# youmi-zym/GO-SLAM

Hardware: AMD Instinct MI355X
Metric: BA keyframes/s (6 x FactorGraph.update: reproject + corr lookup + GRU + 2 GN BA iters) on synthetic 640x480 RGB-D (higher is better)
Workload: dtype f32 (BA/geometry; fp64 solve), f16 (corr volume, GRU convs); 1 GPU; configs[1]-shaped frontend window: 60x80 maps (480x640 RGB-D), P=25 keyframes, E=75 edges, 6 updates/keyframe, iters=2, RGB-D depth prior, upsample on; parallelism=replicas x1 (tracking does not shard)

## Files before the change

go_slam_amd/_lib.py:

```python
import ctypes
import os
import subprocess

_HERE = os.path.dirname(os.path.abspath(__file__))
CSRC = os.path.join(_HERE, "csrc")
LIB_PATH = os.environ.get("GOSLAM_HIP_LIB") or os.path.join(CSRC, "libgoslam_hip.so")

_lib = None

c_int, c_float, c_void_p, c_size_t = ctypes.c_int, ctypes.c_float, ctypes.c_void_p, ctypes.c_size_t

_P = c_void_p
SIGNATURES = {
    "gs_version": (ctypes.c_char_p, []),
    "gs_last_error": (ctypes.c_char_p, []),
    "gs_enc_conv_wpack_elems": (c_size_t, [c_int, c_int, c_int]),
    "gs_enc_conv_stat_chunks": (c_int, [c_int, c_int, c_int]),
    "gs_enc_conv": (c_int, [_P, c_int, c_int, _P, _P, _P, c_int, c_int, c_int, c_int, c_int, c_int, c_int, _P, _P, _P]),
    "gs_norm_act_workspace_bytes_chunks": (c_size_t, [c_int, c_int, c_int]),
    "gs_timing_begin": (c_int, [_P]),
    "gs_timing_end": (c_int, []),
    "gs_timing_read": (c_int, [ctypes.c_char_p, ctypes.POINTER(ctypes.c_double), ctypes.POINTER(c_int)]),
    "gs_timing_names": (c_int, [ctypes.c_char_p, c_int]),
    "gs_corr_index_forward": (c_int, [_P, _P, _P] + [c_int] * 7 + [_P]),
# ... 28 lines not shown
    "gs_upmask_upsample": (c_int, [_P, c_int, _P, _P, _P, _P, _P, c_int, c_int, c_int, _P]),
    "gs_bias_act": (c_int, [_P, _P, _P, c_int, c_int, c_int, c_int, c_int, _P]),
    "gs_motion_features": (c_int, [_P, _P, _P, c_int, c_int, c_int, _P]),
    "gs_ba_inputs": (c_int, [_P] * 6 + [c_int, c_int, c_int, _P]),
    "gs_lowmem_gather": (c_int, [_P] * 7 + [c_int, c_int, c_int, _P]),
    "gs_lowmem_scatter": (c_int, [_P] * 8 + [c_int, c_int, c_int, _P]),
    "gs_damping_rows": (c_int, [_P] * 5 + [c_int, c_int, c_float, c_float, _P]),
    "gs_conv1x1": (c_int, [_P, c_int, c_int, _P, _P, c_int, _P, c_int, c_int, ctypes.c_longlong, _P]),
    "gs_conv7x7_c4": (c_int, [_P, _P, _P, _P, c_int, c_int, c_int, c_int, c_int, c_int, _P]),
    "gs_conv3x3_wpack_elems": (c_size_t, [c_int, c_int]),
    "gs_conv3x3_pp": (c_int, [_P, c_int, c_int, _P, c_int, _P, c_int, c_int, c_int, c_int, c_int, c_int, _P]),
    "gs_conv3x3_bias_relu": (c_int, [_P, c_int, c_int, _P, _P, _P, c_int, c_int, c_int, c_int, c_int, _P]),
    "gs_conv3x3_gru_zr": (c_int, [_P, c_int, c_int, _P, _P, _P, _P, _P, _P, c_int, c_int, c_int, _P]),
    "gs_conv3x3_gru_zr2": (c_int, [_P, _P, c_int, c_int, _P, _P, _P, _P, _P, _P, c_int, c_int, c_int, _P]),
    "gs_conv3x3_gru_q": (c_int, [_P, _P, c_int, c_int, _P, _P, _P, _P, _P, _P, _P, c_int, c_int, c_int, _P]),
    "gs_conv3x3_head": (c_int, [_P, c_int, _P, c_int, _P, _P, c_int, c_int, c_float, _P, c_int, c_int, c_int, _P]),
    "gs_conv3x3_heads": (c_int, [_P, c_int, c_int, _P, c_int, _P, _P, c_int, _P, _P, c_int, c_int, c_int, c_int, c_int, _P]),
    "gs_conv3x3_heads_finish": (c_int, [_P, _P, _P, c_int, c_int, c_float, c_float, _P, _P, c_int, c_int, c_int, _P]),
    "gs_segment_mean": (c_int, [_P, c_int, _P, c_int, _P, _P, _P, c_int, c_int, c_int, _P]),
    "gs_norm_act_workspace_bytes": (c_size_t, [c_int, c_int, c_int]),
    "gs_norm_act": (c_int, [_P, _P, _P, _P] + [c_int] * 6 + [c_float, _P, c_size_t, c_int, _P]),
    "gs_gru_glo_workspace_bytes": (c_size_t, [c_int]),
    "gs_gru_glo": (c_int, [_P] * 11 + [c_int, c_int, _P, c_size_t, _P]),
    "gs_gru_glo_fused_workspace_bytes": (c_size_t, [c_int, c_int]),
    "gs_gru_glo_fused": (c_int, [_P, c_int] + [_P] * 10 + [c_int, c_int, _P, c_size_t, _P]),
    "gs_gru_gate_zr": (c_int, [_P] * 6 + [c_int] * 3 + [_P]),
    "gs_gru_gate_q": (c_int, [_P] * 7 + [c_int] * 2 + [_P]),
    "gs_edge_prep": (c_int, [_P] * 4 + [c_int, _P, _P] + [c_int] * 6 + [c_float, c_int, c_int, _P]),
    "gs_edge_greedy": (c_int, [_P] * 5 + [c_int] * 5 + [c_float, c_int, c_int, _P]),
    "gs_ba_workspace_bytes": (c_size_t, [c_int] * 5),
# ... 179 lines not shown
```

go_slam_amd/csrc/conv3x3_pp.hip:

```cpp
#include "common.h"
#include "conv3x3_common.h"

namespace {

constexpr int PP_KG = 4;
constexpr int PP_PSTR = 5;
constexpr int pp_zpad(int tw) { return (((2 * (tw + 2) + 2) * PP_PSTR + 3 + 15) / 16) * 16; }
constexpr int pp_patch_slots(int tw) {
  return (((512 / tw + 2) * (tw + 2) * PP_PSTR + 511) / 512) * 512 + pp_zpad(tw);
}

__device__ __attribute__((aligned(16))) const uint32_t pp_zero_page[4] = {0u, 0u, 0u, 0u};

__device__ __forceinline__ void pp_glds16(const void* src, void* lds_wave_base) {
  __builtin_amdgcn_global_load_lds((const __attribute__((address_space(1))) void*)src,
                                   (__attribute__((address_space(3))) void*)lds_wave_base, 16, 0, 0);
}

#define PP_BAR()                              \
  do {                                        \
    asm volatile("" ::: "memory");            \
    __builtin_amdgcn_s_barrier();             \
    asm volatile("" ::: "memory");            \
    __builtin_amdgcn_sched_barrier(0);        \
  } while (0)

#define PP_LGKM0()                                        \
  do {                                                    \
    asm volatile("s_waitcnt lgkmcnt(0)" ::: "memory");    \
    __builtin_amdgcn_sched_barrier(0);                    \
  } while (0)

struct PpEpi {
  const float* bias;
  const float* glo;
  const _Float16* inp_pre;
  const _Float16* aux0;
  const _Float16* aux1;
  _Float16* out0;
  _Float16* out1;
  const _Float16* xb;
  int xsb, split;
  const half8* tapw;
  float* tap_out;
  int n_tap;
  long long* dbg;
  int variant;
};

template <bool PROBE>
__device__ __forceinline__ void pp_stamp(long long* dbg, int slot) {
// ... 279 lines not shown
          }
        }
        __builtin_amdgcn_fence(__ATOMIC_RELEASE, "wavefront");
        __builtin_amdgcn_wave_barrier();
      }
      return;
    }
  }
  constexpr int PIECES = NJ * 4;
  constexpr int PXIT = 64 / PIECES;
  constexpr int NIT = 32 / PXIT;
#pragma unroll
  for (int i = 0; i < 4; ++i) {
    size_t pix4[NIT];
    bool ok4[NIT];
    half8 pi4[NIT], u4[NIT], v4[NIT];
    const int piece = lane & (PIECES - 1);
    const int c8 = wn * (PP_BN / 2) + piece * 8;
#pragma unroll
    for (int it = 0; it < NIT; ++it) {
      const int pxr = it * PXIT + lane / PIECES;
      int ty, tx;
      tile_pixel<TW, true>(wm, i, pxr, ty, tx);
      const int gv = g0 + ty, gx = tx0 + tx;
      ok4[it] = gv < rows && gx < W;
      pix4[it] = (size_t)gv * W + gx;
      if constexpr (EPI == 1 || EPI == 2) {
        const half8 z8 = {0, 0, 0, 0, 0, 0, 0, 0};
        pi4[it] = z8; u4[it] = z8; v4[it] = z8;
        if (ok4[it]) {
          if constexpr (EPI == 1) {
            if (ep.inp_pre) pi4[it] = *reinterpret_cast<const half8*>(ep.inp_pre + pix4[it] * 384 + nb * 128 + c8);
            if (nb == 1) u4[it] = *reinterpret_cast<const half8*>(x + pix4[it] * xs + c8);
          } else {
            if (ep.inp_pre) pi4[it] = *reinterpret_cast<const half8*>(ep.inp_pre + pix4[it] * 384 + 256 + c8);
            u4[it] = *reinterpret_cast<const half8*>(ep.aux0 + pix4[it] * 128 + c8);
            v4[it] = *reinterpret_cast<const half8*>(ep.aux1 + pix4[it] * 128 + c8);
          }
        }
      }
    }
#pragma unroll
    for (int j = 0; j < NJ; ++j)
#pragma unroll
      for (int g = 0; g < 4; ++g) {
        half4 o;
#pragma unroll
        for (int e = 0; e < 4; ++e) o[e] = (_Float16)acc[j][i][4 * g + e];
        *reinterpret_cast<half4*>(tile + r * PP_TS + j * 32 + 8 * g + 4 * kgl) = o;
      }
// ... 3 lines not shown
#pragma unroll
    for (int it = 0; it < NIT; ++it) {
      const int pxr = it * PXIT + lane / PIECES;
      if (ok4[it]) {
        const half8 v = *reinterpret_cast<const half8*>(tile + pxr * PP_TS + piece * 8);
        const size_t pix = pix4[it];
        if constexpr (EPI == 0 || EPI == 4) {
          *reinterpret_cast<half8*>(yb + pix * ys + piece * 8) = v;
        } else if constexpr (EPI == 3) {
          const float* bb = ep.bias + nb * PP_BN + c8;
          half8 o;
#pragma unroll
          for (int k = 0; k < 8; ++k) o[k] = (_Float16)fmaxf((float)v[k] + bb[k], 0.0f);
          *reinterpret_cast<half8*>(yb + pix * ys + piece * 8) = o;
        } else if constexpr (EPI == 1) {
          const int img = (int)(pix / ((size_t)H * W));
          const half8 pi = pi4[it];
          const float* bb = ep.bias + nb * 128 + c8;
          const float* gg = ep.glo + (size_t)img * 256 + nb * 128 + c8;
          half8 o;
          if (nb == 0) {
#pragma unroll
            for (int k = 0; k < 8; ++k) o[k] = (_Float16)pp_sigm((float)v[k] + (float)pi[k] + bb[k] + gg[k]);
            *reinterpret_cast<half8*>(ep.out0 + pix * 128 + c8) = o;
          } else {
            const half8 net = u4[it];
#pragma unroll
            for (int k = 0; k < 8; ++k)
              o[k] = (_Float16)(pp_sigm((float)v[k] + (float)pi[k] + bb[k] + gg[k]) * (float)net[k]);
            *reinterpret_cast<half8*>(ep.out1 + pix * 128 + c8) = o;
          }
        } else {
          const int img = (int)(pix / ((size_t)H * W));
          const half8 pi = pi4[it], zz = u4[it], nn = v4[it];
          const float* bb = ep.bias + c8;
          const float* gg = ep.glo + (size_t)img * 128 + c8;
          half8 o;
#pragma unroll
          for (int k = 0; k < 8; ++k) {
            const float a_ = (float)v[k] + (float)pi[k] + bb[k] + gg[k];
            const float q = gs_tanh(a_);
            const float zf = (float)zz[k];
            o[k] = (_Float16)((1.0f - zf) * (float)nn[k] + zf * q);
          }
          *reinterpret_cast<half8*>(ep.out0 + pix * 128 + c8) = o;
        }
      }
    }
// ... 62 lines not shown
  GS_REQUIRE(hx_stride >= c_in && hx_stride % 8 == 0, "conv3x3_gru_zr: bad hx_stride");
  GS_REQUIRE(n >= 0 && h > 0 && w > 0, "conv3x3_gru_zr: bad shape");
  if (n == 0) return GS_OK;
  PpEpi ep = PpEpi();
  ep.bias = bias_zr;
  ep.glo = glo_zr;
  ep.inp_pre = (const _Float16*)inp_pre;
  ep.out0 = (_Float16*)z_out;
  ep.out1 = (_Float16*)rnet_out;
  ep.xb = (const _Float16*)hx;
  ep.xsb = hx_stride;
  ep.split = 1 << 30;
  return dispatch_pp<1>(hx, hx_stride, c_in, wpack, pp_tile_width(w), nullptr, 0, 256, n, h, w, 1, (hipStream_t)stream, ep);
}

extern "C" int gs_conv3x3_gru_zr2(const void* net, const void* x_rest, int x_rest_stride, int c_rest, const void* wpack,
                                  const float* bias_zr, const float* glo_zr, const void* inp_pre, void* z_out,
                                  void* rnet_out, int n, int h, int w, gs_stream_t stream) {
  GS_REQUIRE(net && x_rest && wpack && bias_zr && glo_zr && z_out && rnet_out, "conv3x3_gru_zr2: null pointer");
  GS_REQUIRE(c_rest > 0 && c_rest % 32 == 0, "conv3x3_gru_zr2: c_rest must be a multiple of 32");
  GS_REQUIRE(x_rest_stride >= c_rest && x_rest_stride % 8 == 0, "conv3x3_gru_zr2: bad x_rest_stride");
  GS_REQUIRE(n >= 0 && h > 0 && w > 0, "conv3x3_gru_zr2: bad shape");
  if (n == 0) return GS_OK;
  PpEpi ep = PpEpi();
  ep.bias = bias_zr;
  ep.glo = glo_zr;
  ep.inp_pre = (const _Float16*)inp_pre;
  ep.out0 = (_Float16*)z_out;
  ep.out1 = (_Float16*)rnet_out;
  ep.xb = (const _Float16*)x_rest;
  ep.xsb = x_rest_stride;
  ep.split = 128;
  return dispatch_pp<1>(net, 128, 128 + c_rest, wpack, pp_tile_width(w), nullptr, 0, 256, n, h, w, 1,
                        (hipStream_t)stream, ep);
}

extern "C" int gs_conv3x3_gru_q(const void* rnet, const void* x_rest, int x_rest_stride, int c_rest, const void* wpack,
                                const float* bias_q, const float* glo_q, const void* inp_pre, const void* z,
                                const void* net, void* net_out, int n, int h, int w, gs_stream_t stream) {
  GS_REQUIRE(rnet && x_rest && wpack && bias_q && glo_q && z && net && net_out, "conv3x3_gru_q: null pointer");
  GS_REQUIRE(c_rest > 0 && c_rest % 32 == 0, "conv3x3_gru_q: c_rest must be a multiple of 32");
  GS_REQUIRE(x_rest_stride >= c_rest && x_rest_stride % 8 == 0, "conv3x3_gru_q: bad x_rest_stride");
  GS_REQUIRE(n >= 0 && h > 0 && w > 0, "conv3x3_gru_q: bad shape");
  if (n == 0) return GS_OK;
  PpEpi ep = PpEpi();
  ep.bias = bias_q;
  ep.glo = glo_q;
  ep.inp_pre = (const _Float16*)inp_pre;
  ep.aux0 = (const _Float16*)z;
  ep.aux1 = (const _Float16*)net;
  ep.out0 = (_Float16*)net_out;
  ep.xb = (const _Float16*)x_rest;
  ep.xsb = x_rest_stride;
  ep.split = 128;
  return dispatch_pp<2>(rnet, 128, 128 + c_rest, wpack, pp_tile_width(w), nullptr, 0, 128, n, h, w, 1,
                        (hipStream_t)stream, ep);
}

extern "C" int gs_conv3x3_bias_relu(const void* x, int x_stride, int c_in, const void* wpack, const float* bias, void* y,
                                    int y_stride, int n_out, int n, int h, int w, gs_stream_t stream) {
  GS_REQUIRE(x && wpack && bias && y, "conv3x3_bias_relu: null pointer");
  GS_REQUIRE(c_in > 0 && c_in % 32 == 0, "conv3x3_bias_relu: c_in must be a multiple of 32");
  GS_REQUIRE(n_out > 0 && n_out % 64 == 0, "conv3x3_bias_relu: n_out must be a multiple of 64");
  GS_REQUIRE(x_stride >= c_in && x_stride % 8 == 0, "conv3x3_bias_relu: bad x_stride");
  GS_REQUIRE(y_stride >= n_out && y_stride % 8 == 0, "conv3x3_bias_relu: bad y_stride");
  GS_REQUIRE(n >= 0 && h > 0 && w > 0, "conv3x3_bias_relu: bad shape");
  if (n == 0) return GS_OK;
  PpEpi ep = PpEpi();
  ep.bias = bias;
  if (pp_block_channels(n_out) == 64)
    return dispatch_pp<3, 64>(x, x_stride, c_in, wpack, pp_tile_width(w), y, y_stride, n_out, n, h, w, 1,
// ... 42 lines not shown
```

go_slam_amd/droid_net.py:

```python
import os

import torch
import torch.nn as nn
import torch.nn.functional as F

from .weight_packs import WeightPacks, conv_pack, tensors_key


class GradientClip(nn.Module):

    def forward(self, x):
        return x


def segment_mean(x, index, num_segments):
    n = x.shape[0]
    onehot = torch.zeros(num_segments, n, dtype=x.dtype, device=x.device)
    onehot[index, torch.arange(n, device=x.device)] = 1
    cnt = onehot.sum(dim=1, keepdim=True).clamp(min=1)
    avg = (onehot / cnt)
    if x.is_contiguous(memory_format=torch.channels_last):
        flat = x.permute(0, 2, 3, 1).reshape(n, -1)
        out = (avg @ flat).view(num_segments, x.shape[2], x.shape[3], x.shape[1])
        return out.permute(0, 3, 1, 2)
# ... 146 lines not shown
    c = cy - in_channel if channels is None else channels
    dst, ldy, off = (y, cy, in_channel) if out is None else (out, out.shape[1], out_channel)
    rc = _lib.lib().gs_bias_act(y.data_ptr() + 2 * in_channel, _lib.ptr(b), dst.data_ptr() + 2 * off, n * h * wd, c,
                                cy, ldy, _ACT[act], _lib.stream_ptr(y.device))
    _lib.check(rc, "bias_act")
    return dst


CONV3X3_IMPL = "own"
GRU_FUSED_EPILOGUE = True
CONV7X7_OWN = True
GRU_GLO_FUSED = True
FUSE_UPMASK_UPSAMPLE = True
FUSE_HEAD_TAPS = True
FUSE_LOOKUP_ENCODER = True
_CONV3X3_PACKS = {}
_CONV3X3_PACKS_MAX = 32


def pack_conv3x3_weight(weight, kc=32):
    O, C, kh, kw = weight.shape
    bn = 128 if O % 128 == 0 else 64
    assert (kh, kw) == (3, 3) and O % bn == 0 and C % kc == 0 and kc == 32
    w = weight.detach().half().reshape(O // bn, bn, C // kc, kc // 8, 8, 3, 3)
    return w.permute(0, 2, 5, 6, 3, 1, 4).contiguous().reshape(-1)


def conv3x3_hip_supported(x, w):
    return (x.is_cuda and x.dtype == torch.float16 and x.dim() == 4 and tuple(w.shape[2:]) == (3, 3)
            and w.shape[0] % 64 == 0 and w.shape[1] % 32 == 0 and x.shape[1] == w.shape[1]
            and x.is_contiguous(memory_format=torch.channels_last))

# ... 175 lines not shown
            ws = torch.empty(L.gs_gru_glo_fused_workspace_bytes(b, hw), dtype=torch.uint8, device=dev)
            _lib.check(L.gs_gru_glo_fused(_lib.ptr(net), 128, _lib.ptr(ww_pack), _lib.ptr(bw), _lib.ptr(gw[0]),
                                          _lib.ptr(gw[1]), _lib.ptr(gw[2]), _lib.ptr(gw[3]), _lib.ptr(gw[4]),
                                          _lib.ptr(gw[5]), _lib.ptr(gzr), _lib.ptr(gq), b, hw, _lib.ptr(ws),
                                          ws.numel(), st), "gru_glo_fused")
        else:
            w_pre = torch.empty_like(net)
            _lib.check(L.gs_conv1x1(_lib.ptr(net), 128, 128, _lib.ptr(ww_pack), None, 0, _lib.ptr(w_pre), 128,
                                    128, b * hw, st), "conv1x1(gru.w)")
            ws = torch.empty(L.gs_gru_glo_workspace_bytes(b), dtype=torch.uint8, device=dev)
            _lib.check(L.gs_gru_glo(_lib.ptr(w_pre), _lib.ptr(bw), _lib.ptr(net), _lib.ptr(gw[0]), _lib.ptr(gw[1]),
                                    _lib.ptr(gw[2]), _lib.ptr(gw[3]), _lib.ptr(gw[4]), _lib.ptr(gw[5]),
                                    _lib.ptr(gzr), _lib.ptr(gq), b, hw, _lib.ptr(ws), ws.numel(), st), "gru_glo")
        return gzr, gq

    def forward_hx(self, net, hx, inp_pre=None, glo=None):
        from . import _lib
        b, c, h, w = net.shape
        hw = h * w
        (wzr, wq, bzr, bq, ww, bw, gw), hoist, _ = self._all_packs()
        if inp_pre is not None:
            wzr, wq = hoist[1], hoist[2]
        L = _lib.lib()
        st = _lib.stream_ptr(net.device)
        dev = net.device
        with torch.autocast("cuda", enabled=False):
            gzr, gq = glo if glo is not None else self.global_context(net)
            cin = hx.shape[1]
            if GRU_FUSED_EPILOGUE and _use_own_conv3x3(hx, wzr, 1, 1) and h * w > 0:
                z = torch.empty_like(net)
                rnet = torch.empty_like(net)
                out = torch.empty_like(net)
                _lib.check(L.gs_conv3x3_gru_zr2(_lib.ptr(net), hx.data_ptr() + 2 * 128, cin, cin - 128,
                                                _lib.ptr(conv3x3_weight_image(wzr, 32)), _lib.ptr(bzr), _lib.ptr(gzr),
                                                _lib.ptr(inp_pre), _lib.ptr(z), _lib.ptr(rnet), b, h, w, st),
                           "conv3x3_gru_zr2")
                _lib.check(L.gs_conv3x3_gru_q(_lib.ptr(rnet), hx.data_ptr() + 2 * 128, cin, cin - 128,
                                              _lib.ptr(conv3x3_weight_image(wq, 32)), _lib.ptr(bq), _lib.ptr(gq),
                                              _lib.ptr(inp_pre), _lib.ptr(z), _lib.ptr(net), _lib.ptr(out), b, h, w,
                                              st), "conv3x3_gru_q")
                return out
            copy_channels(net, hx, 0)
            zr_pre = conv_nobias(hx, wzr, padding=1)
            z = torch.empty_like(net)
            _lib.check(L.gs_gru_gate_zr(_lib.ptr(zr_pre), _lib.ptr(bzr), _lib.ptr(gzr), _lib.ptr(inp_pre), _lib.ptr(hx),
                                        _lib.ptr(z), b, hw, hx.shape[1], st), "gru_gate_zr")
            q_pre = conv_nobias(hx, wq, padding=1)
            out = torch.empty_like(net)
            _lib.check(L.gs_gru_gate_q(_lib.ptr(q_pre), _lib.ptr(bq), _lib.ptr(gq), _lib.ptr(inp_pre), _lib.ptr(z),
                                       _lib.ptr(net), _lib.ptr(out), b, hw, st), "gru_gate_q")
        return out

    def forward(self, net, *inputs):
        if self.fuse_gates and self._fusable(net, inputs):
            return self._forward_fused(net, inputs)
        inp = torch.cat(inputs, dim=1)
# ... 73 lines not shown

    def _cache_cap(self, device):
        cap = self.INP_CACHE_BYTES
        if device.type == "cuda":
            idx = device.index if device.index is not None else torch.cuda.current_device()
            dev_cap = UpdateModule._device_caps.get(idx)
            if dev_cap is None:
                try:
                    dev_cap = torch.cuda.mem_get_info(device)[1] // 8
                except RuntimeError:
                    dev_cap = cap
                UpdateModule._device_caps[idx] = dev_cap
            cap = min(cap, dev_cap)
        return cap

    def _edge_state(self, inp, n, ht, wd):
        import collections
        import weakref
        hx = getattr(self, "_hx", None)
        if hx is None or hx.shape[0] != n or hx.shape[2:] != (ht, wd) or hx.device != inp.device:
            hx = torch.empty((n, 320, ht, wd), dtype=torch.float16, device=inp.device,
                             memory_format=torch.channels_last)
            self._hx = hx
        cache = getattr(self, "_inp_pre_cache", None)
        if cache is None:
            cache = self._inp_pre_cache = collections.OrderedDict()
        wkey = self.gru._weights_key()
        owner = inp._base if inp._base is not None else inp
        key = (inp.data_ptr(), tuple(inp.shape), tuple(inp.stride()), inp.dtype)
        ent = cache.get(key)
        if ent is not None and ent[0]() is owner and ent[1] == inp._version and ent[2] == wkey:
            if self.cache_check and ent[4] != self._checksum(inp):
                raise RuntimeError("UpdateModule: the context features `inp` were modified behind the version counter "
                                   "(raw-pointer write?) while their hoisted convolution was cached; call "
                                   "update.invalidate_context() after such writes")
            cache.move_to_end(key)
            return hx, ent[3]
        inp4 = inp.view(n, -1, ht, wd)
        if inp4.dtype != torch.float16 or not inp4.is_contiguous(memory_format=torch.channels_last):
            inp4 = inp4.half().contiguous(memory_format=torch.channels_last)
        try:
            inp_pre = self.gru.inp_gates(inp4)
        except torch.OutOfMemoryError:
            cache.clear()
            torch.cuda.empty_cache()
            inp_pre = self.gru.inp_gates(inp4)
        for k in [k for k, e in cache.items() if e[2] != wkey or e[0]() is None]:
            del cache[k]

        def _gone(_ref, key=key, cache_ref=weakref.ref(cache)):
            c = cache_ref()
            if c is not None:
                e = c.get(key)
                if e is not None and e[0] is _ref:
                    del c[key]
        cache[key] = (weakref.ref(owner, _gone), inp._version, wkey, inp_pre,
                      self._checksum(inp) if self.cache_check else None)
        nbytes = lambda e: sum(x.numel() * x.element_size()
                               for x in (e[3] if isinstance(e[3], (tuple, list)) else (e[3],)) if torch.is_tensor(x))
        total = sum(nbytes(e) for e in cache.values())
        cap = self._cache_cap(inp.device)
# ... 24 lines not shown
    def _heads_workspace(self, n, ht, wd, n_out, device):
        ws = self.__dict__.setdefault("_heads_ws", {})
        key = (n, ht, wd, n_out, device)
        hit = ws.pop(key, None)
        if hit is None:
            ts, rs = heads_workspace_shapes(n, ht, wd, n_out, 2)
            taps = torch.empty(ts, dtype=torch.float32, device=device)
            rest = None if rs is None else torch.empty((n, rs[3], ht, wd), dtype=torch.float16, device=device,
                                                       memory_format=torch.channels_last)
            hit = (taps, rest)
            while len(ws) >= self.HEADS_WS_ENTRIES:
                ws.pop(next(iter(ws)))
        ws[key] = hit
        return hit

    def _corr_independent_part(self, net4, inp, f4, n, ht, wd):
        hx, inp_pre = self._edge_state(inp, n, ht, wd)
        if CONV7X7_OWN and conv7x7_c4_supported(self.flow_encoder[0], f4):
            f4 = conv7x7_c4_bias_act(self._packs, self.flow_encoder[0], f4, "relu")
        else:
            f4 = conv_bias_act(self._packs, self.flow_encoder[0], f4, "relu")
        conv_bias_act(self._packs, self.flow_encoder[2], f4, "relu", out=hx, out_channel=256)
        with torch.autocast("cuda", enabled=False):
            glo = self.gru.global_context(net4)
        return hx, inp_pre, glo

    def _forward_fast(self, net, inp, corr, flow, ii, jj, seg=None):
        batch, num, ch, ht, wd = net.shape
        cl = torch.channels_last
        packs = self._packs
        out_dim = (batch, num, -1, ht, wd)
        n = batch * num
        net4 = net.view(n, -1, ht, wd)
        from .corr import LazyLookup
        lazy = corr if isinstance(corr, LazyLookup) and FUSE_LOOKUP_ENCODER and corr.block.fused_encoder_supported() \
            else None
        if lazy is None:
            if isinstance(corr, LazyLookup):
                corr = corr.materialize()
            c4 = corr.view(n, -1, ht, wd).half().contiguous(memory_format=cl)
        if flow is None:
            flow = torch.zeros(batch, num, 4, ht, wd, device=net.device)
        f4 = flow.view(n, -1, ht, wd).half().contiguous(memory_format=cl)
        hx, inp_pre, glo = self._corr_independent_part(net4, inp, f4, n, ht, wd)
        if lazy is not None:
            c4 = lazy.encoded(*self._corr_enc0_padded())
        else:
            c4 = conv1x1_bias_act(packs, self.corr_encoder[0], c4, "relu")
        conv_bias_act(packs, self.corr_encoder[2], c4, "relu", out=hx, out_channel=128)
        net4 = self.gru.forward_hx(net4, hx, inp_pre, glo=glo)
        net = net4.view(*out_dim)
        hw_, hb = self._head_weights()
        hw_ = hw_ if ii is not None else hw_[:256]
        fused = FUSE_HEAD_TAPS and _use_own_conv3x3(net4, hw_, 1, 1)
        if fused:
            tapw, tapb, b_delta, b_weight = self._head_taps()
            taps, heads = self._heads_workspace(n, ht, wd, hw_.shape[0], net4.device)
            delta, weight = conv3x3_heads_fused(net4, hw_, tapw, tapb, taps, heads, b_delta, b_weight)
            agg_channel = 0
        else:
            heads = conv_nobias(net4, hw_, padding=1)
            delta = conv3x3_head(heads, self.delta[2], packs, "none", in_channel=0, in_bias=hb[0], in_relu=True)
            weight = conv3x3_head(heads, self.weight[2], packs, "sigmoid", in_channel=128, in_bias=hb[1], in_relu=True)
            agg_channel = 256
        delta, weight = delta.view(batch, num, ht, wd, 2), weight.view(batch, num, ht, wd, 2)
# ... 12 lines not shown
        return net, delta, weight, eta, upmask

    def _corr_enc0_padded(self):
        def pad(weight):
            w = torch.zeros(128, 208, dtype=torch.float16, device=weight.device)
            w[:, :196] = weight.detach().reshape(128, 196).half()
            return w
        return conv_pack(self._packs, self.corr_encoder[0], "pad208", pad)

    def _fast_ok(self, net, inp, corr):
        cl = torch.channels_last
        n4 = net.view(-1, *net.shape[2:])
        return (self.fuse_epilogues and net.is_cuda and not torch.is_grad_enabled() and net.dtype == torch.float16
                and net.shape[2] == 128 and n4.is_contiguous(memory_format=cl) and torch.is_autocast_enabled())

    def forward(self, net, inp, corr, flow=None, ii=None, jj=None, seg=None):
        batch, num, ch, ht, wd = net.shape
        if self._fast_ok(net, inp, corr):
            return self._forward_fast(net, inp, corr, flow, ii, jj, seg)
        if hasattr(corr, "materialize"):
            corr = corr.materialize()
        if flow is None:
            flow = torch.zeros(batch, num, 4, ht, wd, device=net.device)
        out_dim = (batch, num, -1, ht, wd)
        net = net.view(batch * num, -1, ht, wd)
        inp = inp.view(batch * num, -1, ht, wd)
        corr = self.corr_encoder(corr.view(batch * num, -1, ht, wd))
        flow = self.flow_encoder(flow.view(batch * num, -1, ht, wd))
        net = self.gru(net, inp, corr, flow)
        delta = self.delta(net).view(*out_dim).permute(0, 1, 3, 4, 2)[..., :2].contiguous()
        weight = self.weight(net).view(*out_dim).permute(0, 1, 3, 4, 2)[..., :2].contiguous()
        net = net.view(*out_dim)
        if ii is not None:
            eta, upmask = self.agg(net, ii.to(net.device))
# ... 23 lines not shown
```

go_slam_amd/factor_graph.py:

```python
import numpy as np
import torch

from .corr import AltCorrBlock, CorrBlock, CorrPool

def coords_grid(ht, wd, device):
    y, x = torch.meshgrid(torch.arange(ht, device=device).float(), torch.arange(wd, device=device).float(),
                          indexing="ij")
    return torch.stack([x, y], dim=-1)


def _segments_np(index):
    uniq, ix = np.unique(index, return_inverse=True)
    ix = ix.reshape(-1).astype(np.int64)
    order = np.argsort(ix, kind="stable").astype(np.int32)
    offsets = np.zeros(uniq.size + 1, dtype=np.int32)
    offsets[1:] = np.cumsum(np.bincount(ix, minlength=uniq.size))
    return {"uniq": uniq.astype(np.int64), "ix": ix, "offsets": offsets, "order": order, "n": int(uniq.size)}


def _as_tensors(d):
    return {k: (torch.from_numpy(np.ascontiguousarray(v)) if isinstance(v, np.ndarray) else v) for k, v in d.items()}


def upload_tables(host, device):
# ... 73 lines not shown
            up["sel"] = np.nonzero(m)[0].astype(np.int64)
            ii_all = np.concatenate([iin[m], ii_c])
            up["ii"] = ii_all
            up["jj"] = np.concatenate([jin[m], jj_c])
        else:
            c["ii"], c["jj"] = self.ii.contiguous(), self.jj.contiguous()
        dindex = np.unique(np.concatenate([np.arange(a0, a1, dtype=np.int64), ii_all]))
        up["damping_index"] = dindex
        uniq = seg_h["uniq"]
        if uniq.size:
            pos = np.minimum(np.searchsorted(uniq, dindex), uniq.size - 1)
            inv = np.where(uniq[pos] == dindex, pos, -1)
        else:
            inv = np.full(dindex.shape, -1)
        up["damping_inv"] = inv.astype(np.int32)
        up = upload_tables(_as_tensors(up), dev)
        c["seg"] = {k: (up["seg." + k] if isinstance(v, np.ndarray) else v) for k, v in seg_h.items()}
        for k in ("sel", "ii", "jj", "damping_index", "damping_inv"):
            if k in up:
                c[k] = up[k]
        uniq = torch.from_numpy(uniq)
        c["uniq_host"] = uniq
        self._eidx = c
        return c

    def _glue_fusable(self, coords1):
        return coords1.is_cuda and self.channels_last and self.target.dtype == torch.float32 \
            and self.target.is_contiguous() and coords1.is_contiguous()

    def _ba_buffers(self, idx, use_inactive):
        if "ba_target" not in idx:
            ht, wd = self.ht, self.wd
            E = self.ii.numel()
            if use_inactive and idx["sel"].numel():
                ti = self.target_inac[0, idx["sel"]].permute(0, 3, 1, 2)
                wi = self.weight_inac[0, idx["sel"]].permute(0, 3, 1, 2)
            else:
                ti = wi = torch.zeros(0, 2, ht, wd, device=self.device)
            n_in = ti.shape[0]
# ... 235 lines not shown
        fused = self._glue_fusable(coords1)
        ht, wd = self.ht, self.wd
        E = self.ii.numel()
        if fused:
            from . import _lib
            L, st = _lib.lib(), _lib.stream_ptr(self.device)
            m4 = torch.empty(E, ht, wd, 4, dtype=torch.float16, device=self.device)
            _lib.check(L.gs_motion_features(_lib.ptr(coords1), _lib.ptr(self.target), _lib.ptr(m4), E, ht, wd, st),
                       "motion_features")
            motion = m4.permute(0, 3, 1, 2).unsqueeze(0)
        else:
            motion = torch.cat([coords1 - self.coords0, self.target - coords1], dim=-1)
            motion = motion.permute(0, 1, 4, 2, 3).clamp(-64.0, 64.0)

        corr = self.corr.lazy(coords1) if hasattr(self.corr, "lazy") else self.corr(coords1)
        with torch.autocast("cuda", dtype=torch.float16):
            self.net, delta, weight, damping, upmask = self.update_op(
                self.net, self.inp, corr, motion, self.ii, self.jj, seg=seg)

        fuse_damping = fused and damping.dtype == torch.float32 and damping.is_contiguous() and \
            self.damping.is_contiguous() and damping.shape[1] == idx["uniq_host"].numel()
        if not fuse_damping:
            self.damping[seg["uniq"]] = damping.float()
        eta_rows = damping
        if fused and delta.dtype == torch.float32 and weight.dtype == torch.float32:
            bt, bw, n_in = self._ba_buffers(idx, use_inactive)
            target_new = torch.empty_like(coords1)
            _lib.check(L.gs_ba_inputs(_lib.ptr(coords1), _lib.ptr(delta.contiguous()), _lib.ptr(weight.contiguous()),
                                      _lib.ptr(target_new), bt[n_in:].data_ptr(), bw[n_in:].data_ptr(), E, ht, wd, st),
                       "ba_inputs")
            self.target, self.weight = target_new, weight
            target, weight = bt, bw
        else:
# ... 45 lines not shown
        a0 = max(1, int(ii_c.min()) + 1) if t0 is None else t0
        a0 = max(1, a0)
        a1 = (max(int(ii_c.max()), int(jj_c.max())) + 1) if t1 is None else t1
        chunks, up, segs = [], {}, []
        s = 13
        for i in range(int(ii_c.min()), int(ii_c.max()) + 1, s):
            sel = np.nonzero((ii_c >= i) & (ii_c < i + s))[0].astype(np.int64)
            if sel.size < 1:
                continue
            iis, jjs = ii_c[sel], jj_c[sel]
            n = len(segs)
            up.update({f"{n}.sel": sel, f"{n}.ii": iis, f"{n}.jj": jjs, f"{n}.corr_ii": rig * iis,
                       f"{n}.corr_jj": rig * jjs + (iis == jjs).astype(np.int64), f"{n}.uniq": np.unique(iis)})
            segs.append(_segments_np(iis))
            up.update({f"{n}.seg.{k}": v for k, v in segs[-1].items() if isinstance(v, np.ndarray)})
        up["damping_index"] = np.unique(np.concatenate([np.arange(a0, a1, dtype=np.int64), ii_c]))
        up = _as_tensors(up)
        up = upload_tables(up, dev)
        for n, seg_h in enumerate(segs):
            ck = {k: up[f"{n}.{k}"] for k in ("sel", "ii", "jj", "corr_ii", "corr_jj", "uniq")}
            seg = {k: (up[f"{n}.seg.{k}"] if isinstance(v, np.ndarray) else v) for k, v in seg_h.items()}
            ck["seg_kw"] = {"seg": seg} if getattr(self.update_op, "_forward_fast", None) is not None else {}
            def _inp(ix=ck["ii"], box=ck):
                v = box.get("inp_cached")
                if v is None:
                    v = box["inp_cached"] = self._fmt(self.video.inps[ix]).unsqueeze(0)
                return v
            ck["inp"] = _inp
            chunks.append(ck)
        c = {"key": key, "tens": tens, "t0": a0, "t1": a1, "chunks": chunks, "ii": self.ii.contiguous(),
             "jj": self.jj.contiguous(), "damping_index": up["damping_index"]}
        self._lidx = c
        return c

    @torch.no_grad()
    def update_lowmem(self, t0=None, t1=None, iters=2, use_inactive=False, EPS=1e-7, steps=8, max_t=None,
                      ba_type="dense", motion_only=False):
        cur_t = self.video.counter
        cur_t = int(getattr(cur_t, "value", cur_t))
        t = max_t if max_t is not None else cur_t
        fm = self.video.fmaps[:cur_t + 2]
        num, rig, ch, ht, wd = fm.shape
        corr_op = AltCorrBlock(fm.reshape(1, num * rig, ch, ht, wd))
# ... 21 lines not shown
                sel, iis, jjs = ck["sel"], ck["ii"], ck["jj"]
                if fast:
                    n = sel.numel()
                    c1 = torch.empty(1, n, ht, wd, 2, dtype=torch.float32, device=self.device)
                    m4 = torch.empty(n, ht, wd, 4, dtype=torch.float16, device=self.device)
                    net_c = torch.empty(n, ht, wd, 128, dtype=torch.float16, device=self.device)
                    _lib.check(L.gs_lowmem_gather(_lib.ptr(coords1), _lib.ptr(self.target), _lib.ptr(self.net),
                                                  _lib.ptr(sel), _lib.ptr(c1), _lib.ptr(m4), _lib.ptr(net_c), n, ht, wd, st),
                               "lowmem_gather")
                    net_in = net_c.permute(0, 3, 1, 2).unsqueeze(0)
                    motion_c = m4.permute(0, 3, 1, 2).unsqueeze(0)
                else:
                    c1 = coords1.index_select(1, sel)
                    net_in, motion_c = self._select_edges(self.net, sel), motion.index_select(1, sel)
                corr1 = lookup(c1, ck["corr_ii"], ck["corr_jj"])
                with torch.autocast("cuda", dtype=torch.float16):
                    net, delta, weight, damping, upmask = self.update_op(
                        net_in, ck["inp"](), corr1, motion_c, iis, jjs, **ck["seg_kw"])
                    if self.upsample:
                        self.video.upsample(ck["uniq"], upmask[0])
                if fast and net.dtype == torch.float16 and net[0].is_contiguous(memory_format=cl) \
                        and tuple(net.shape) == (1, sel.numel(), 128, ht, wd) \
                        and delta.dtype == torch.float32 and weight.dtype == torch.float32 \
                        and tuple(delta.shape) == tuple(weight.shape) == (1, sel.numel(), ht, wd, 2):
                    delta_c, weight_c = delta.contiguous(), weight.contiguous()
                    _lib.check(L.gs_lowmem_scatter(_lib.ptr(c1), _lib.ptr(delta_c), _lib.ptr(weight_c),
                                                   _lib.ptr(net), _lib.ptr(sel), _lib.ptr(self.target), _lib.ptr(self.weight),
                                                   _lib.ptr(self.net), sel.numel(), ht, wd, st), "lowmem_scatter")
                else:
                    self.net[:, sel] = net.to(self.net.dtype)
                    self.target[:, sel] = c1 + delta.float()
                    self.weight[:, sel] = weight.float()
                self.damping[ck["uniq"]] = damping.float()
# ... 9 lines not shown
```

include/goslam_hip.h:

```cpp
#ifndef GOSLAM_HIP_H
#define GOSLAM_HIP_H

#include <stddef.h>
#include <stdint.h>

#ifdef __cplusplus
extern "C" {
#endif

typedef void* gs_stream_t;

typedef enum {
  GS_OK = 0,
  GS_ERR_INVALID_ARG = -1,
  GS_ERR_WORKSPACE = -2,
  GS_ERR_LAUNCH = -3,
  GS_ERR_UNSUPPORTED = -4
} gs_status;

typedef enum { GS_F16 = 0, GS_F32 = 1, GS_F64 = 2 } gs_dtype;

const char* gs_version(void);
const char* gs_last_error(void);

// ... 131 lines not shown
                  int rt, gs_stream_t stream);
size_t gs_conv3x3_wpack_elems(int c_in, int n_out);
int gs_conv3x3_pp(const void* x, int x_stride, int c_in, const void* wpack, int tw, void* y, int y_stride, int n_out,
                  int n, int h, int w, int xcd_order, gs_stream_t stream);
int gs_conv3x3_bias_relu(const void* x, int x_stride, int c_in, const void* wpack, const float* bias, void* y,
                         int y_stride, int n_out, int n, int h, int w, gs_stream_t stream);
int gs_conv3x3_gru_zr2(const void* net, const void* x_rest, int x_rest_stride, int c_rest, const void* wpack,
                       const float* bias_zr, const float* glo_zr, const void* inp_pre, void* z_out, void* rnet_out,
                       int n, int h, int w, gs_stream_t stream);
int gs_conv3x3_gru_zr(const void* hx, int hx_stride, int c_in, const void* wpack, const float* bias_zr,
                      const float* glo_zr, const void* inp_pre, void* z_out, void* rnet_out, int n, int h, int w,
                      gs_stream_t stream);
int gs_conv3x3_gru_q(const void* rnet, const void* x_rest, int x_rest_stride, int c_rest, const void* wpack,
                     const float* bias_q, const float* glo_q, const void* inp_pre, const void* z, const void* net,
                     void* net_out, int n, int h, int w, gs_stream_t stream);
int gs_conv3x3_head(const void* x, int x_stride, const float* in_bias, int in_relu, const void* wpack,
                    const float* bias, int n_out, int epilogue, float out_scale, float* out, int n, int h, int w,
                    gs_stream_t stream);
int gs_conv3x3_heads(const void* x, int x_stride, int c_in, const void* wpack, int tw, const void* tap_wpack,
                     const float* in_bias, int n_tap_blocks, float* tap_out, void* y, int y_stride, int n_out, int n,
                     int h, int w, gs_stream_t stream);
int gs_conv3x3_heads_finish(const float* tap, const float* bias0, const float* bias1, int epilogue0, int epilogue1,
                            float out_scale0, float out_scale1, float* out0, float* out1, int n, int h, int w,
                            gs_stream_t stream);
int gs_segment_mean(const void* x, int x_stride, const float* in_bias, int in_relu, const int* seg_offsets,
                    const int* seg_edges, void* out, int n_seg, int hw, int channels, gs_stream_t stream);
size_t gs_norm_act_workspace_bytes(int n, int hw, int channels);
size_t gs_norm_act_workspace_bytes_chunks(int n, int chunks, int channels);
size_t gs_enc_conv_wpack_elems(int ksize, int c_in, int c_out);
int gs_enc_conv_stat_chunks(int h_out, int w_out, int c_out);
// ... 65 lines not shown
```

Baseline: 84.52 keyframes/s.

## Compute GRU context gates once per keyframe and index them per edge

The hoisted context-gate convolution (inp_gates) now runs on the unique source keyframes' context features instead of on a per-edge gathered copy. The fused GRU zr/q epilogues take an int32 edge-to-keyframe index and read the 384-channel precomputed term from the matching keyframe row. This removes the gather of the context tensor and the redundant convolution over duplicate keyframes (E=75 edges vs far fewer unique sources). In exchange it adds index plumbing, extra cache-key handling and indirect loads in the epilogue.

```diff
diff --git a/go_slam_amd/_lib.py b/go_slam_amd/_lib.py
--- a/go_slam_amd/_lib.py
+++ b/go_slam_amd/_lib.py
@@ -66,6 +66,9 @@
     "gs_conv3x3_gru_zr": (c_int, [_P, c_int, c_int, _P, _P, _P, _P, _P, _P, c_int, c_int, c_int, _P]),
     "gs_conv3x3_gru_zr2": (c_int, [_P, _P, c_int, c_int, _P, _P, _P, _P, _P, _P, c_int, c_int, c_int, _P]),
     "gs_conv3x3_gru_q": (c_int, [_P, _P, c_int, c_int, _P, _P, _P, _P, _P, _P, _P, c_int, c_int, c_int, _P]),
+    "gs_conv3x3_gru_zr2_src": (c_int, [_P, _P, c_int, c_int, _P, _P, _P, _P, _P, c_int, _P, _P, c_int, c_int, c_int, _P]),
+    "gs_conv3x3_gru_q_src": (c_int, [_P, _P, c_int, c_int, _P, _P, _P, _P, _P, c_int, _P, _P, _P, c_int, c_int, c_int,
+                                     _P]),
     "gs_conv3x3_head": (c_int, [_P, c_int, _P, c_int, _P, _P, c_int, c_int, c_float, _P, c_int, c_int, c_int, _P]),
     "gs_conv3x3_heads": (c_int, [_P, c_int, c_int, _P, c_int, _P, _P, c_int, _P, _P, c_int, c_int, c_int, c_int, c_int, _P]),
     "gs_conv3x3_heads_finish": (c_int, [_P, _P, _P, c_int, c_int, c_float, c_float, _P, _P, c_int, c_int, c_int, _P]),
diff --git a/go_slam_amd/csrc/conv3x3_pp.hip b/go_slam_amd/csrc/conv3x3_pp.hip
--- a/go_slam_amd/csrc/conv3x3_pp.hip
+++ b/go_slam_amd/csrc/conv3x3_pp.hip
@@ -35,6 +35,7 @@
   const float* bias;
   const float* glo;
   const _Float16* inp_pre;
+  const int* inp_src;
   const _Float16* aux0;
   const _Float16* aux1;
   _Float16* out0;
@@ -344,6 +345,7 @@
   for (int i = 0; i < 4; ++i) {
     size_t pix4[NIT];
     bool ok4[NIT];
+    [[maybe_unused]] int img4[NIT];
     half8 pi4[NIT], u4[NIT], v4[NIT];
     const int piece = lane & (PIECES - 1);
     const int c8 = wn * (PP_BN / 2) + piece * 8;
@@ -358,12 +360,19 @@
       if constexpr (EPI == 1 || EPI == 2) {
         const half8 z8 = {0, 0, 0, 0, 0, 0, 0, 0};
         pi4[it] = z8; u4[it] = z8; v4[it] = z8;
+        img4[it] = 0;
         if (ok4[it]) {
+          img4[it] = gv / H;
+          size_t ipix = pix4[it];
+          if (ep.inp_src) {
+            const size_t img0 = (size_t)img4[it] * H * W;
+            ipix = (size_t)ep.inp_src[img4[it]] * H * W + (pix4[it] - img0);
+          }
           if constexpr (EPI == 1) {
-            if (ep.inp_pre) pi4[it] = *reinterpret_cast<const half8*>(ep.inp_pre + pix4[it] * 384 + nb * 128 + c8);
+            if (ep.inp_pre) pi4[it] = *reinterpret_cast<const half8*>(ep.inp_pre + ipix * 384 + nb * 128 + c8);
             if (nb == 1) u4[it] = *reinterpret_cast<const half8*>(x + pix4[it] * xs + c8);
           } else {
-            if (ep.inp_pre) pi4[it] = *reinterpret_cast<const half8*>(ep.inp_pre + pix4[it] * 384 + 256 + c8);
+            if (ep.inp_pre) pi4[it] = *reinterpret_cast<const half8*>(ep.inp_pre + ipix * 384 + 256 + c8);
             u4[it] = *reinterpret_cast<const half8*>(ep.aux0 + pix4[it] * 128 + c8);
             v4[it] = *reinterpret_cast<const half8*>(ep.aux1 + pix4[it] * 128 + c8);
           }
@@ -397,7 +406,7 @@
           for (int k = 0; k < 8; ++k) o[k] = (_Float16)fmaxf((float)v[k] + bb[k], 0.0f);
           *reinterpret_cast<half8*>(yb + pix * ys + piece * 8) = o;
         } else if constexpr (EPI == 1) {
-          const int img = (int)(pix / ((size_t)H * W));
+          const int img = img4[it];
           const half8 pi = pi4[it];
           const float* bb = ep.bias + nb * 128 + c8;
           const float* gg = ep.glo + (size_t)img * 256 + nb * 128 + c8;
@@ -414,7 +423,7 @@
             *reinterpret_cast<half8*>(ep.out1 + pix * 128 + c8) = o;
           }
         } else {
-          const int img = (int)(pix / ((size_t)H * W));
+          const int img = img4[it];
           const half8 pi = pi4[it], zz = u4[it], nn = v4[it];
           const float* bb = ep.bias + c8;
           const float* gg = ep.glo + (size_t)img * 128 + c8;
@@ -507,9 +516,9 @@
   return dispatch_pp<1>(hx, hx_stride, c_in, wpack, pp_tile_width(w), nullptr, 0, 256, n, h, w, 1, (hipStream_t)stream, ep);
 }
 
-extern "C" int gs_conv3x3_gru_zr2(const void* net, const void* x_rest, int x_rest_stride, int c_rest, const void* wpack,
-                                  const float* bias_zr, const float* glo_zr, const void* inp_pre, void* z_out,
-                                  void* rnet_out, int n, int h, int w, gs_stream_t stream) {
+static int gru_zr2(const void* net, const void* x_rest, int x_rest_stride, int c_rest, const void* wpack,
+                   const float* bias_zr, const float* glo_zr, const void* inp_pre, const int* inp_src, void* z_out,
+                   void* rnet_out, int n, int h, int w, gs_stream_t stream) {
   GS_REQUIRE(net && x_rest && wpack && bias_zr && glo_zr && z_out && rnet_out, "conv3x3_gru_zr2: null pointer");
   GS_REQUIRE(c_rest > 0 && c_rest % 32 == 0, "conv3x3_gru_zr2: c_rest must be a multiple of 32");
   GS_REQUIRE(x_rest_stride >= c_rest && x_rest_stride % 8 == 0, "conv3x3_gru_zr2: bad x_rest_stride");
@@ -519,6 +528,7 @@
   ep.bias = bias_zr;
   ep.glo = glo_zr;
   ep.inp_pre = (const _Float16*)inp_pre;
+  ep.inp_src = inp_src;
   ep.out0 = (_Float16*)z_out;
   ep.out1 = (_Float16*)rnet_out;
   ep.xb = (const _Float16*)x_rest;
@@ -528,9 +538,26 @@
                         (hipStream_t)stream, ep);
 }
 
-extern "C" int gs_conv3x3_gru_q(const void* rnet, const void* x_rest, int x_rest_stride, int c_rest, const void* wpack,
-                                const float* bias_q, const float* glo_q, const void* inp_pre, const void* z,
-                                const void* net, void* net_out, int n, int h, int w, gs_stream_t stream) {
+extern "C" int gs_conv3x3_gru_zr2(const void* net, const void* x_rest, int x_rest_stride, int c_rest, const void* wpack,
+                                  const float* bias_zr, const float* glo_zr, const void* inp_pre, void* z_out,
+                                  void* rnet_out, int n, int h, int w, gs_stream_t stream) {
+  return gru_zr2(net, x_rest, x_rest_stride, c_rest, wpack, bias_zr, glo_zr, inp_pre, nullptr, z_out, rnet_out, n, h, w,
+                 stream);
+}
+
+extern "C" int gs_conv3x3_gru_zr2_src(const void* net, const void* x_rest, int x_rest_stride, int c_rest,
+                                      const void* wpack, const float* bias_zr, const float* glo_zr, const void* inp_pre,
+                                      const int* inp_src, int n_src, void* z_out, void* rnet_out, int n, int h, int w,
+                                      gs_stream_t stream) {
+  GS_REQUIRE(inp_pre && inp_src, "conv3x3_gru_zr2_src: null context term or index");
+  GS_REQUIRE(n_src > 0, "conv3x3_gru_zr2_src: n_src must be positive");
+  return gru_zr2(net, x_rest, x_rest_stride, c_rest, wpack, bias_zr, glo_zr, inp_pre, inp_src, z_out, rnet_out, n, h, w,
+                 stream);
+}
+
+static int gru_q(const void* rnet, const void* x_rest, int x_rest_stride, int c_rest, const void* wpack,
+                 const float* bias_q, const float* glo_q, const void* inp_pre, const int* inp_src, const void* z,
+                 const void* net, void* net_out, int n, int h, int w, gs_stream_t stream) {
   GS_REQUIRE(rnet && x_rest && wpack && bias_q && glo_q && z && net && net_out, "conv3x3_gru_q: null pointer");
   GS_REQUIRE(c_rest > 0 && c_rest % 32 == 0, "conv3x3_gru_q: c_rest must be a multiple of 32");
   GS_REQUIRE(x_rest_stride >= c_rest && x_rest_stride % 8 == 0, "conv3x3_gru_q: bad x_rest_stride");
@@ -540,6 +567,7 @@
   ep.bias = bias_q;
   ep.glo = glo_q;
   ep.inp_pre = (const _Float16*)inp_pre;
+  ep.inp_src = inp_src;
   ep.aux0 = (const _Float16*)z;
   ep.aux1 = (const _Float16*)net;
   ep.out0 = (_Float16*)net_out;
@@ -548,6 +576,23 @@
   ep.split = 128;
   return dispatch_pp<2>(rnet, 128, 128 + c_rest, wpack, pp_tile_width(w), nullptr, 0, 128, n, h, w, 1,
                         (hipStream_t)stream, ep);
+}
+
+extern "C" int gs_conv3x3_gru_q(const void* rnet, const void* x_rest, int x_rest_stride, int c_rest, const void* wpack,
+                                const float* bias_q, const float* glo_q, const void* inp_pre, const void* z,
+                                const void* net, void* net_out, int n, int h, int w, gs_stream_t stream) {
+  return gru_q(rnet, x_rest, x_rest_stride, c_rest, wpack, bias_q, glo_q, inp_pre, nullptr, z, net, net_out, n, h, w,
+               stream);
+}
+
+extern "C" int gs_conv3x3_gru_q_src(const void* rnet, const void* x_rest, int x_rest_stride, int c_rest, const void* wpack,
+                                    const float* bias_q, const float* glo_q, const void* inp_pre, const int* inp_src,
+                                    int n_src, const void* z, const void* net, void* net_out, int n, int h, int w,
+                                    gs_stream_t stream) {
+  GS_REQUIRE(inp_pre && inp_src, "conv3x3_gru_q_src: null context term or index");
+  GS_REQUIRE(n_src > 0, "conv3x3_gru_q_src: n_src must be positive");
+  return gru_q(rnet, x_rest, x_rest_stride, c_rest, wpack, bias_q, glo_q, inp_pre, inp_src, z, net, net_out, n, h, w,
+               stream);
 }
 
 extern "C" int gs_conv3x3_bias_relu(const void* x, int x_stride, int c_in, const void* wpack, const float* bias, void* y,
diff --git a/go_slam_amd/droid_net.py b/go_slam_amd/droid_net.py
--- a/go_slam_amd/droid_net.py
+++ b/go_slam_amd/droid_net.py
@@ -184,8 +184,36 @@
 FUSE_UPMASK_UPSAMPLE = True
 FUSE_HEAD_TAPS = True
 FUSE_LOOKUP_ENCODER = True
+CONTEXT_PER_KEYFRAME = True
 _CONV3X3_PACKS = {}
 _CONV3X3_PACKS_MAX = 32
+
+
+def context_per_keyframe_active():
+    return CONTEXT_PER_KEYFRAME and GRU_FUSED_EPILOGUE and CONV3X3_IMPL == "own"
+
+
+class ContextSource:
+
+    def __init__(self, ctx, index, index_host=None):
+        import numpy as np
+        if ctx is None or index is None:
+            raise ValueError("ContextSource: ctx and index are required")
+        self.ctx = ctx if ctx.dim() == 5 else ctx.unsqueeze(0)
+        n_src = self.ctx.shape[1]
+        host = index_host if index_host is not None else (index.cpu() if torch.is_tensor(index) else index)
+        host = np.asarray(host).reshape(-1)
+        if host.size and (int(host.min()) < 0 or int(host.max()) >= n_src):
+            raise ValueError(f"ContextSource: index values must lie in [0, {n_src})")
+        if not torch.is_tensor(index):
+            index = torch.from_numpy(host.astype(np.int32))
+        if index.numel() != host.size:
+            raise ValueError("ContextSource: index and index_host differ in length")
+        self.index = index.to(device=self.ctx.device, dtype=torch.int32).reshape(-1).contiguous()
+        self.n_src = int(n_src)
+
+    def gathered(self):
+        return self.ctx.index_select(1, self.index.long())
 
 
 def pack_conv3x3_weight(weight, kc=32):
@@ -391,7 +419,7 @@
                                     _lib.ptr(gzr), _lib.ptr(gq), b, hw, _lib.ptr(ws), ws.numel(), st), "gru_glo")
         return gzr, gq
 
-    def forward_hx(self, net, hx, inp_pre=None, glo=None):
+    def forward_hx(self, net, hx, inp_pre=None, glo=None, inp_src=None):
         from . import _lib
         b, c, h, w = net.shape
         hw = h * w
@@ -408,6 +436,23 @@
                 z = torch.empty_like(net)
                 rnet = torch.empty_like(net)
                 out = torch.empty_like(net)
+                if inp_src is not None:
+                    if inp_pre is None or inp_src.dtype != torch.int32 or inp_src.device != net.device \
+                            or inp_src.numel() != b or not inp_src.is_contiguous() \
+                            or tuple(inp_pre.shape[1:]) != (384, h, w):
+                        raise ValueError("ConvGRU.forward_hx: inp_src must be a contiguous int32 [b] on net's device "
+                                         "and inp_pre [n_src,384,h,w]")
+                    n_src = inp_pre.shape[0]
+                    _lib.check(L.gs_conv3x3_gru_zr2_src(_lib.ptr(net), hx.data_ptr() + 2 * 128, cin, cin - 128,
+                                                        _lib.ptr(conv3x3_weight_image(wzr, 32)), _lib.ptr(bzr),
+                                                        _lib.ptr(gzr), _lib.ptr(inp_pre), _lib.ptr(inp_src), n_src,
+                                                        _lib.ptr(z), _lib.ptr(rnet), b, h, w, st),
+                               "conv3x3_gru_zr2_src")
+                    _lib.check(L.gs_conv3x3_gru_q_src(_lib.ptr(rnet), hx.data_ptr() + 2 * 128, cin, cin - 128,
+                                                      _lib.ptr(conv3x3_weight_image(wq, 32)), _lib.ptr(bq), _lib.ptr(gq),
+                                                      _lib.ptr(inp_pre), _lib.ptr(inp_src), n_src, _lib.ptr(z),
+                                                      _lib.ptr(net), _lib.ptr(out), b, h, w, st), "conv3x3_gru_q_src")
+                    return out
                 _lib.check(L.gs_conv3x3_gru_zr2(_lib.ptr(net), hx.data_ptr() + 2 * 128, cin, cin - 128,
                                                 _lib.ptr(conv3x3_weight_image(wzr, 32)), _lib.ptr(bzr), _lib.ptr(gzr),
                                                 _lib.ptr(inp_pre), _lib.ptr(z), _lib.ptr(rnet), b, h, w, st),
@@ -417,6 +462,9 @@
                                               _lib.ptr(inp_pre), _lib.ptr(z), _lib.ptr(net), _lib.ptr(out), b, h, w,
                                               st), "conv3x3_gru_q")
                 return out
+            if inp_src is not None:
+                raise RuntimeError("ConvGRU.forward_hx: the per-keyframe context term (inp_src) needs the fused gate "
+                                   "epilogues; pass the gathered term instead")
             copy_channels(net, hx, 0)
             zr_pre = conv_nobias(hx, wzr, padding=1)
             z = torch.empty_like(net)
@@ -520,9 +568,13 @@
             cap = min(cap, dev_cap)
         return cap
 
-    def _edge_state(self, inp, n, ht, wd):
+    def _edge_state(self, inp, n, ht, wd, source=None):
         import collections
         import weakref
+        if source is not None:
+            inp, n_img = source.ctx, source.n_src
+        else:
+            n_img = n
         hx = getattr(self, "_hx", None)
         if hx is None or hx.shape[0] != n or hx.shape[2:] != (ht, wd) or hx.device != inp.device:
             hx = torch.empty((n, 320, ht, wd), dtype=torch.float16, device=inp.device,
@@ -534,6 +586,8 @@
         wkey = self.gru._weights_key()
         owner = inp._base if inp._base is not None else inp
         key = (inp.data_ptr(), tuple(inp.shape), tuple(inp.stride()), inp.dtype)
+        if source is not None:
+            key += ("per_keyframe",)
         ent = cache.get(key)
         if ent is not None and ent[0]() is owner and ent[1] == inp._version and ent[2] == wkey:
             if self.cache_check and ent[4] != self._checksum(inp):
@@ -541,8 +595,10 @@
                                    "(raw-pointer write?) while their hoisted convolution was cached; call "
                                    "update.invalidate_context() after such writes")
             cache.move_to_end(key)
+            if source is not None and ent[3][1] is not source.index:
+                ent = cache[key] = ent[:3] + ((ent[3][0], source.index),) + ent[4:]
             return hx, ent[3]
-        inp4 = inp.view(n, -1, ht, wd)
+        inp4 = inp.view(n_img, -1, ht, wd)
         if inp4.dtype != torch.float16 or not inp4.is_contiguous(memory_format=torch.channels_last):
             inp4 = inp4.half().contiguous(memory_format=torch.channels_last)
         try:
@@ -551,6 +607,8 @@
             cache.clear()
             torch.cuda.empty_cache()
             inp_pre = self.gru.inp_gates(inp4)
+        if source is not None:
+            inp_pre = (inp_pre, source.index)
         for k in [k for k, e in cache.items() if e[2] != wkey or e[0]() is None]:
             del cache[k]
 
@@ -605,8 +663,9 @@
         ws[key] = hit
         return hit
 
-    def _corr_independent_part(self, net4, inp, f4, n, ht, wd):
-        hx, inp_pre = self._edge_state(inp, n, ht, wd)
+    def _corr_independent_part(self, net4, inp, f4, n, ht, wd, source=None):
+        hx, inp_pre = self._edge_state(inp, n, ht, wd, source)
+        inp_pre, inp_src = inp_pre if source is not None else (inp_pre, None)
         if CONV7X7_OWN and conv7x7_c4_supported(self.flow_encoder[0], f4):
             f4 = conv7x7_c4_bias_act(self._packs, self.flow_encoder[0], f4, "relu")
         else:
@@ -614,9 +673,9 @@
         conv_bias_act(self._packs, self.flow_encoder[2], f4, "relu", out=hx, out_channel=256)
         with torch.autocast("cuda", enabled=False):
             glo = self.gru.global_context(net4)
-        return hx, inp_pre, glo
-
-    def _forward_fast(self, net, inp, corr, flow, ii, jj, seg=None):
+        return hx, inp_pre, inp_src, glo
+
+    def _forward_fast(self, net, inp, corr, flow, ii, jj, seg=None, inp_source=None):
         batch, num, ch, ht, wd = net.shape
         cl = torch.channels_last
         packs = self._packs
@@ -633,13 +692,17 @@
         if flow is None:
             flow = torch.zeros(batch, num, 4, ht, wd, device=net.device)
         f4 = flow.view(n, -1, ht, wd).half().contiguous(memory_format=cl)
-        hx, inp_pre, glo = self._corr_independent_part(net4, inp, f4, n, ht, wd)
+        if inp_source is not None and inp_source.index.numel() != n:
+            raise ValueError("UpdateModule: inp_source.index must hold one row per edge")
+        if inp_source is not None and not context_per_keyframe_active():
+            inp, inp_source = (inp if inp is not None else inp_source.gathered()), None
+        hx, inp_pre, inp_src, glo = self._corr_independent_part(net4, inp, f4, n, ht, wd, inp_source)
         if lazy is not None:
             c4 = lazy.encoded(*self._corr_enc0_padded())
         else:
             c4 = conv1x1_bias_act(packs, self.corr_encoder[0], c4, "relu")
         conv_bias_act(packs, self.corr_encoder[2], c4, "relu", out=hx, out_channel=128)
-        net4 = self.gru.forward_hx(net4, hx, inp_pre, glo=glo)
+        net4 = self.gru.forward_hx(net4, hx, inp_pre, glo=glo, inp_src=inp_src)
         net = net4.view(*out_dim)
         hw_, hb = self._head_weights()
         hw_ = hw_ if ii is not None else hw_[:256]
@@ -682,10 +745,12 @@
         return (self.fuse_epilogues and net.is_cuda and not torch.is_grad_enabled() and net.dtype == torch.float16
                 and net.shape[2] == 128 and n4.is_contiguous(memory_format=cl) and torch.is_autocast_enabled())
 
-    def forward(self, net, inp, corr, flow=None, ii=None, jj=None, seg=None):
+    def forward(self, net, inp, corr, flow=None, ii=None, jj=None, seg=None, inp_source=None):
         batch, num, ch, ht, wd = net.shape
         if self._fast_ok(net, inp, corr):
-            return self._forward_fast(net, inp, corr, flow, ii, jj, seg)
+            return self._forward_fast(net, inp, corr, flow, ii, jj, seg, inp_source)
+        if inp is None:
+            inp = inp_source.gathered()
         if hasattr(corr, "materialize"):
             corr = corr.materialize()
         if flow is None:
diff --git a/go_slam_amd/factor_graph.py b/go_slam_amd/factor_graph.py
--- a/go_slam_amd/factor_graph.py
+++ b/go_slam_amd/factor_graph.py
@@ -111,15 +111,33 @@
         else:
             inv = np.full(dindex.shape, -1)
         up["damping_inv"] = inv.astype(np.int32)
+        c["inp_src_host"] = seg_h["ix"].astype(np.int32)
+        up["inp_src"] = c["inp_src_host"]
         up = upload_tables(_as_tensors(up), dev)
         c["seg"] = {k: (up["seg." + k] if isinstance(v, np.ndarray) else v) for k, v in seg_h.items()}
-        for k in ("sel", "ii", "jj", "damping_index", "damping_inv"):
+        for k in ("sel", "ii", "jj", "damping_index", "damping_inv", "inp_src"):
             if k in up:
                 c[k] = up[k]
         uniq = torch.from_numpy(uniq)
         c["uniq_host"] = uniq
         self._eidx = c
         return c
+
+    def _source_form_ok(self):
+        from .droid_net import context_per_keyframe_active
+        return context_per_keyframe_active() and getattr(self.update_op, "_forward_fast", None) is not None \
+            and torch.is_tensor(getattr(self.video, "inps", None))
+
+    def _context_source(self, idx):
+        if self.inp is None or not self._source_form_ok():
+            return None
+        ver = self.video.inps._version
+        src = idx.get("inp_source")
+        if src is None or src[1] != ver:
+            from .droid_net import ContextSource
+            ctx = self._fmt(self.video.inps[idx["seg"]["uniq"]]).unsqueeze(0)
+            src = idx["inp_source"] = (ContextSource(ctx, idx["inp_src"], index_host=idx["inp_src_host"]), ver)
+        return src[0]
 
     def _glue_fusable(self, coords1):
         return coords1.is_cuda and self.channels_last and self.target.dtype == torch.float32 \
@@ -385,9 +403,11 @@
             motion = motion.permute(0, 1, 4, 2, 3).clamp(-64.0, 64.0)
 
         corr = self.corr.lazy(coords1) if hasattr(self.corr, "lazy") else self.corr(coords1)
+        source = self._context_source(idx)
+        src_kw = {} if source is None else {"inp_source": source}
         with torch.autocast("cuda", dtype=torch.float16):
             self.net, delta, weight, damping, upmask = self.update_op(
-                self.net, self.inp, corr, motion, self.ii, self.jj, seg=seg)
+                self.net, self.inp, corr, motion, self.ii, self.jj, seg=seg, **src_kw)
 
         fuse_damping = fused and damping.dtype == torch.float32 and damping.is_contiguous() and \
             self.damping.is_contiguous() and damping.shape[1] == idx["uniq_host"].numel()
@@ -463,6 +483,7 @@
                        f"{n}.corr_jj": rig * jjs + (iis == jjs).astype(np.int64), f"{n}.uniq": np.unique(iis)})
             segs.append(_segments_np(iis))
             up.update({f"{n}.seg.{k}": v for k, v in segs[-1].items() if isinstance(v, np.ndarray)})
+            up[f"{n}.inp_src"] = segs[-1]["ix"].astype(np.int32)
         up["damping_index"] = np.unique(np.concatenate([np.arange(a0, a1, dtype=np.int64), ii_c]))
         up = _as_tensors(up)
         up = upload_tables(up, dev)
@@ -476,6 +497,15 @@
                     v = box["inp_cached"] = self._fmt(self.video.inps[ix]).unsqueeze(0)
                 return v
             ck["inp"] = _inp
+
+            def _source(box=ck, index=up[f"{n}.inp_src"], host=seg_h["ix"]):
+                v = box.get("source_cached")
+                if v is None:
+                    from .droid_net import ContextSource
+                    ctx = self._fmt(self.video.inps[box["uniq"]]).unsqueeze(0)
+                    v = box["source_cached"] = ContextSource(ctx, index, index_host=host)
+                return v
+            ck["source"] = _source
             chunks.append(ck)
         c = {"key": key, "tens": tens, "t0": a0, "t1": a1, "chunks": chunks, "ii": self.ii.contiguous(),
              "jj": self.jj.contiguous(), "damping_index": up["damping_index"]}
@@ -527,9 +557,10 @@
                     c1 = coords1.index_select(1, sel)
                     net_in, motion_c = self._select_edges(self.net, sel), motion.index_select(1, sel)
                 corr1 = lookup(c1, ck["corr_ii"], ck["corr_jj"])
+                inp_kw = {"inp_source": ck["source"]()} if self._source_form_ok() else {}
                 with torch.autocast("cuda", dtype=torch.float16):
                     net, delta, weight, damping, upmask = self.update_op(
-                        net_in, ck["inp"](), corr1, motion_c, iis, jjs, **ck["seg_kw"])
+                        net_in, None if inp_kw else ck["inp"](), corr1, motion_c, iis, jjs, **ck["seg_kw"], **inp_kw)
                     if self.upsample:
                         self.video.upsample(ck["uniq"], upmask[0])
                 if fast and net.dtype == torch.float16 and net[0].is_contiguous(memory_format=cl) \
diff --git a/include/goslam_hip.h b/include/goslam_hip.h
--- a/include/goslam_hip.h
+++ b/include/goslam_hip.h
@@ -169,6 +169,12 @@
 int gs_conv3x3_gru_q(const void* rnet, const void* x_rest, int x_rest_stride, int c_rest, const void* wpack,
                      const float* bias_q, const float* glo_q, const void* inp_pre, const void* z, const void* net,
                      void* net_out, int n, int h, int w, gs_stream_t stream);
+int gs_conv3x3_gru_zr2_src(const void* net, const void* x_rest, int x_rest_stride, int c_rest, const void* wpack,
+                           const float* bias_zr, const float* glo_zr, const void* inp_pre, const int* inp_src, int n_src,
+                           void* z_out, void* rnet_out, int n, int h, int w, gs_stream_t stream);
+int gs_conv3x3_gru_q_src(const void* rnet, const void* x_rest, int x_rest_stride, int c_rest, const void* wpack,
+                         const float* bias_q, const float* glo_q, const void* inp_pre, const int* inp_src, int n_src,
+                         const void* z, const void* net, void* net_out, int n, int h, int w, gs_stream_t stream);
 int gs_conv3x3_head(const void* x, int x_stride, const float* in_bias, int in_relu, const void* wpack,
                     const float* bias, int n_out, int epilogue, float out_scale, float* out, int n, int h, int w,
                     gs_stream_t stream);
```

New measurement: 83.32 keyframes/s. -1.4%, worse.
